# lowrank/aniso

Measured on AMD Instinct MI355X. Metric: GMRES matvec/s at 1M quad points (aniso.m block matvec, g=0.8, 45 mode-applies), higher is better.
Workload: dtype f64

## Files before the change

aniso_amd/csrc/aniso_op.hip:

```cpp
#include <algorithm>
#include <cmath>
#include <cstdlib>
#include <cstring>
#include <stdexcept>
#include <thread>

#include "aniso_op.hpp"
#include "kernels.hpp"

namespace aniso {

[[noreturn]] void throw_hip(hipError_t e, const char* file, int line) {
    throw std::runtime_error(std::string("HIP error ") + hipGetErrorName(e) + " (" + hipGetErrorString(e) + ") at " +
                             file + ":" + std::to_string(line));
}

#define HIP_CHECK(x)                                         \
    do {                                                     \
        hipError_t e__ = (x);                                \
        if (e__ != hipSuccess) throw_hip(e__, __FILE__, __LINE__); \
    } while (0)

DevBuf::~DevBuf() {
    if (p) (void)hipFree(p);
// ... 947 lines not shown
                      cf.Wc.as<double>(), cf.Wm.as<double>(), P};
    const int ntier = (int)plan.upTierTask.size() - 1;
    const bool upPartial = call.exch.oneX && call.exch.upPartial && phase != 0;
    const bool topFused = harmonic && (mask & kStageFar) && topFusedOn() && !upPartial && !win;
    const bool ringOn = hmRing > 0 && hm_ring_xl(K, plan.hmMaxLds, hmRing) >= 0;
    const bool hsSym = harmonic && plan.nearSymHsOn;
    const bool nearFused = topFused && overlapOn() && nearInTop && !ringOn && !hsSym && plan.nearCorrOk &&
                           near_hs_fusable((int)plan.leaves.size(), plan.nearMaxLeaf, plan.nsMax,
                                           dNearLoc.as<uint16_t>(), &nc, mask);
    const bool fork = harmonic && overlapOn() && !nearFused;
    const hipStream_t sn = fork ? side : s;
    const bool nearIn = harmonic && nearEarly && !nearFused && plan.nearCorrOk && (mask & kStageNear) &&
                        near_hs_fusable((int)plan.leaves.size(), plan.nearMaxLeaf, plan.nsMax,
                                        dNearLoc.as<uint16_t>(), &nc, mask);
    const bool oneX = call.exch.oneX && phase != 0;
    if (oneX && !(harmonic && nearIn))
        throw std::logic_error("one-collective exchange: the apply is not the harmonic one with its near field from the input");
    double* const fTw = nearIn ? nullptr : dFT.as<double>();
    double* const cTw = nearIn ? nullptr : dCT.as<double>();
    const int forkTier = phase == 0 && !topFused ? std::max(ntier - 1, 0) : plan.upLastLeafTier;
    UpTail tail;
    if (upPartial && call.exch.upTails) {
        tail.partOf = dXT0Part.as<int2>();
        const size_t sb = plan.xUpRoots.size() * 16 * kRank * K * sizeof(double);
        if (dXUpStage.bytes < sb) dXUpStage.alloc(sb);
        tail.stage = dXUpStage.as<double>();
        tail.cnt = dXUpCnt.as<unsigned>();
        tail.nroots = dXUpRoots.as<int>();
        tail.task = dXUpTask.as<int>();
        tail.rec = dXUpRec.as<double>();
        tail.nPeer = (int)oxRootParts;
        tail.peerOff = dOxRootSend.as<int64_t>();
        tail.buf = dOxSendBuf.as<double>();
    }
    auto upTier = [&](int k, const int* list, int ntask, const double* recv, double* send, const UpTail* tl = nullptr) {
        launch_up_tier(K, ntask, plan.upTierTask[k], list, plan.upTierMaxTask[k], dUpDesc.as<int4>(), dUpGrpFix.as<int>(),
                       dUpNode.as<int>(), dUpCode.as<int4>(), dUpGeom.as<double4>(), dUpLeaf.as<int2>(),
                       dPxT.as<double>(), dPyT.as<double>(), x, ldx, treeIn ? 1 : 0, dPerm.as<int>(), sigT,
                       dWT.as<double>(), fTw, cTw, P, dMult.as<double>(),
                       recv ? dXRootSlot.as<int>() : nullptr, recv, send ? dXSendSlot.as<int>() : nullptr, send, s,
                       topFused && k == 0 ? dTopCnt.as<unsigned>() : nullptr, tl);
        if (fork && !nearIn && k == forkTier) HIP_CHECK(hipEventRecord(evFork, s));
    };
    auto tierTasks = [&](int k) { return plan.upTierTask[k + 1] - plan.upTierTask[k]; };
    NearHsArgs nin{};
    if (nearIn) {
        nin.xin = x;
        nin.ldi = ldx;
        nin.treeIn = treeIn ? 1 : 0;
        nin.perm = dPerm.as<int>();
        nin.sigT = sigT;
        nin.wT = dWT.as<double>();
    }
    const bool nearUp = phase == 0 && nearIn && !fork && nearUpTier() && ntier >= 1 && !hsSym && K <= 5;
    if (nearUp) {
        nin.upMult = dMult.as<double>();
        nin.upGrp = dNearUpGrp.as<int>();
        nin.upP = P;
        nin.upNcx = dNcx.as<double>();
        nin.upNcy = dNcy.as<double>();
        nin.upNrx = dNrx.as<double>();
        nin.upNry = dNry.as<double>();
        nin.zeroCnt = topFused ? dTopCnt.as<unsigned>() : nullptr;
    }
    if (hsSym) {
        nin.nearSym = dHsSym.as<int2>();
        nin.colDst = dHsDst.as<int>();
        nin.selfRow = dNearSelfRow.as<uint16_t>();
        nin.nearPart = dNearPart.as<double>();
        nin.grpInPtr = dNearGrpInPtr.as<int>();
        nin.grpIn = dNearGrpIn.as<int>();
        nin.grpSlots = plan.nearGrpSlots;
    }
    const int64_t* const hmPtsPtr = (hsSym ? dHsPtsPtr : dNearPtsPtr).as<int64_t>();
    const int64_t* const hmKOff = (hsSym ? dHsKOff : dNearKOff).as<int64_t>();
    const uint16_t* const hmLoc = (hsSym ? dHsLoc : dNearLoc).as<uint16_t>();
    auto nearStage = [&] {
        if (fork) HIP_CHECK(hipStreamWaitEvent(side, evFork, 0));
        const int en = tr ? mark(sn) : -1;
        bool corrFused = false;
        if (harmonic) {
            corrFused = launch_near_hm(K, (int)plan.leaves.size(), plan.nearMaxLeaf, dLeafInfo.as<int4>(), hmPtsPtr,
                           dNearPts.as<int>(), hmKOff, dAttNear.as<double>(), dPxT.as<double>(), dPyT.as<double>(),
                           dSigDiag.as<double>(), hw, dFT.as<double>(), operm, obase, ldo, mask, scale, out, hmLoc,
                           dNsPtr.as<int64_t>(), dNsPts.as<int>(), plan.nsMax, plan.nearCorrOk ? &nc : nullptr,
                           nearWpe, sn, &nin, win);
        } else if (plan.nearPartTotal > 0) {
            for (int t = 0; t < nterm; ++t) {
                const int id = ids[t];
                const double sgn = (id % 2 == 0) ? 1.0 : -1.0;
                launch_near_sym(K, (int)plan.leaves.size(), dLeafInfo.as<int4>(), dNearPtsPtr.as<int64_t>(),
                                dNearPts.as<int>(), dNearKOff.as<int64_t>(), dNearSym.as<int2>(),
                                modes[id].Knear.as<double>(), dFT.as<double>(), mixes + (size_t)t * K * K, operm,
                                obase, ldo, maxNearS, mask, sgn, scale, t > 0 ? 1 : 0, dNearPart.as<double>(), out, s);
            }
        } else {
            launch_near(K, (int)plan.leaves.size(), plan.nearMaxLeaf, dLeafInfo.as<int4>(), dNearPtsPtr.as<int64_t>(),
                        dNearPts.as<int>(), dNearKOff.as<int64_t>(), tab, nterm, dFT.as<double>(), operm, obase, ldo,
                        mask, scale, 0, out, s);
        }
        const int e1 = tr ? mark(sn) : -1;
        span(4, en, e1);
        if (!corrFused)
            launch_corr(K, geo.d, plan.ownBegin, plan.ownEnd, dPerm.as<int>(), dIperm.as<int>(), dCT.as<double>(),
                        dFT.as<double>(), cf.Wc.as<double>(), cf.Wm.as<double>(), P, mask, scale, treeOut, ldo, out, sn);
        const int e2 = tm ? mark(sn) : -1;
        span(6, e1, e2);
        if (fork) HIP_CHECK(hipEventRecord(evJoin, side));
    };
    const bool clustered = harmonic && useClusters && !win;
    const int ncl = (int)plan.hmClPtr.size() - 1;
    HcArgs hca{dHmClPtr.as<int>(), dHmTgt.as<int>(), dHmPtr.as<int64_t>(), dHmNDir.as<int>(), dHmSrc.as<int>(),
                     dHmBlk.as<int>(), dHmSlot.as<int>(), dAttM2L.as<double>(), dNcx.as<double>(), dNcy.as<double>(),
                     dNrx.as<double>(), dNry.as<double>(), P, hw, dMult.as<double>(), dLocal.as<double>(),
                     dNodeGeo.as<double>()};
    hca.wpe = hmWpe;
    const bool halo = !plan.hmHaloNode.empty();
    if (halo) {
        const size_t hb = plan.hmHaloNode.size() * kRank * K * sizeof(double);
        if (dHmPart.bytes < hb) dHmPart.alloc(hb);
        hca.haloPtr = dHmHaloPtr.as<int>();
        hca.haloPos = dHmHaloPos.as<int>();
        hca.hpart = dHmPart.as<double>();
    }
    if (hmRing > 0) {
// ... 1871 lines not shown
```

aniso_amd/csrc/harmonic.hip:

```cpp
#include <hip/hip_runtime.h>

#include <algorithm>
#include <cstdlib>
#include <stdexcept>
#include <string>

#include "corr_point.hpp"
#include "device_common.hpp"
#include "hm_entry.hpp"
#include "up_task.hpp"

namespace aniso {

__device__ __forceinline__ double uniform_f64(double v) {
    const long long b = __double_as_longlong(v);
    const int lo = __builtin_amdgcn_readfirstlane((int)(b & 0xffffffffll));
    const int hi = __builtin_amdgcn_readfirstlane((int)(b >> 32));
    return __longlong_as_double(((long long)hi << 32) | (unsigned)lo);
}

__device__ __forceinline__ int xcd_tile(int bid, int nb) {
    const int x = bid & 7, per = nb >> 3, rem = nb & 7, j = bid >> 3;
    return x < rem ? x * (per + 1) + j : rem * (per + 1) + (x - rem) * per + j;
}
// ... 697 lines not shown
    __syncthreads();
    const bool ok = done != 0;
    __syncthreads();
    return ok;
}

template <int K>
__device__ __forceinline__ void top_ensure(const TopArgs& t, const UpArgs& u, int k, double* sm) {
    int j = k;
    while (j >= 1 && !top_poll(t, j, (unsigned)(t.blk0[j + 1] - t.blk0[j]))) --j;
    for (int jj = j + 1; jj <= k; ++jj) {
        const int nj = t.blk0[jj + 1] - t.blk0[jj];
        for (int i = 0; i < nj; ++i) {
            up_task<K>(t.task0[jj] + i, u.maxTask, u.desc, u.grpFix, u.node, u.code, u.geom, u.leafRange, u.pxT,
                       u.pyT, u.xin, u.ldi, u.treeIn, u.perm, u.sigT, u.wT, u.fT, u.cT, u.P, u.mult, u.rootSlot,
                       jj == 1 ? t.recv1 : nullptr, nullptr, nullptr, sm);
            asm volatile("s_waitcnt vmcnt(0)" ::: "memory");
            __syncthreads();
        }
        if (threadIdx.x == 0 && t.steals)
            __hip_atomic_fetch_add((gu32*)t.steals, (unsigned)nj, __ATOMIC_RELAXED, __HIP_MEMORY_SCOPE_AGENT);
    }
}

__device__ __forceinline__ void top_publish(unsigned* cnt, int k) {
    asm volatile("s_waitcnt vmcnt(0)" ::: "memory");
    __syncthreads();
    if (threadIdx.x == 0) {
        __builtin_amdgcn_fence(__ATOMIC_RELEASE, "agent");
        asm volatile("s_waitcnt vmcnt(0)" ::: "memory");
        __hip_atomic_fetch_add((gu32*)(cnt + k), 1u, __ATOMIC_RELAXED, __HIP_MEMORY_SCOPE_AGENT);
    }
}

template <bool TRACE>
__device__ __forceinline__ void top_mark(const TopArgs& t, int field) {
    if constexpr (!TRACE) return;
    __syncthreads();
    if (threadIdx.x == 0) {
        int64_t* r = t.trace + 4 * (int64_t)blockIdx.x;
        r[field] = (int64_t)__builtin_amdgcn_s_memrealtime();
        if (field == 0)
            r[3] = (int64_t)__builtin_amdgcn_s_getreg((4) | (0 << 6) | (31 << 11)) |
                   ((int64_t)__builtin_amdgcn_s_getreg((20) | (0 << 6) | (3 << 11)) << 32);
    }
}

template <int K, int NR, int D, bool XL, bool LR = false>
__device__ __forceinline__ void m2l_cluster_form(int cid, const HcArgs& a, double* sm) {
    if constexpr (D == 0) m2l_hc_cluster<K, NR, LR>(cid, a, sm);
    else m2l_hcr_cluster<K, NR, D, XL>(cid, a, sm);
}

template <int K, int U, int NR, bool FUSE, bool SYM = false, bool UP = false, bool OFF = false>
__device__ __forceinline__ void near_hs_group(int g, const NearHsArgs& n, double* tab, int i0 = 0, int b0 = 0);

template <int K, int NR, int WPE, int D, bool XL, bool TRACE = false, bool NEAR = false>
__global__ void __launch_bounds__(kHcThreads<WPE>) __attribute__((amdgpu_waves_per_eu(kHcWaves<WPE>)))
k_top_m2l_hc(UpArgs u, TopArgs t, HcArgs a, NearHsArgs n) {
    extern __shared__ double sm[];
    const int b = (int)blockIdx.x;
    top_mark<TRACE>(t, 0);
    if (b < t.nUp) {
        int k = 1;
        while (b >= t.blk0[k + 1]) ++k;
        if (k >= 2) top_ensure<K>(t, u, k - 1, sm);
        top_mark<TRACE>(t, 1);
        up_task<K>(t.task0[k] + (b - t.blk0[k]), u.maxTask, u.desc, u.grpFix, u.node, u.code, u.geom, u.leafRange,
                   u.pxT, u.pyT, u.xin, u.ldi, u.treeIn, u.perm, u.sigT, u.wT, u.fT, u.cT, u.P, u.mult, u.rootSlot,
                   k == 1 ? t.recv1 : nullptr, nullptr, nullptr, sm);
        top_publish(t.cnt, k);
        top_mark<TRACE>(t, 2);
        return;
    }
    const int cid = b - t.nUp;
    if constexpr (NEAR) {
        if (cid >= t.nCl) {
            top_mark<TRACE>(t, 1);
            near_hs_group<K, 4, 2, true>(cid - t.nCl, n, sm);
            top_mark<TRACE>(t, 2);
            return;
        }
    }
    const int w = t.clWait[cid];
    if (w > 0) {
        top_ensure<K>(t, u, w, sm);
        top_mark<TRACE>(t, 1);
        m2l_cluster_form<K, NR, D, XL, kHcLR<WPE>>(cid, a, sm);
        top_mark<TRACE>(t, 2);
        return;
    }
    top_mark<TRACE>(t, 1);
    m2l_cluster_form<K, NR, D, XL, kHcLR<WPE>>(cid, a, sm);
    top_mark<TRACE>(t, 2);
}


template <int K, int G, int U, int NR, bool XCD = false, bool OFF = false>
__global__ void __launch_bounds__(256) k_near_hm(int nl, const int4* __restrict__ leafInfo,
                                                 const int64_t* __restrict__ nearPtsPtr,
                                                 const int* __restrict__ nearPts, const int64_t* __restrict__ nearKOff,
                                                 const double* __restrict__ E, const double* __restrict__ pxT,
                                                 const double* __restrict__ pyT, const double* __restrict__ sigDiag,
                                                 HarmArg<OFF> hw, const double* __restrict__ fT,
                                                 const int* __restrict__ operm, int64_t obase, int64_t ldo,
                                                 int flags, double scale, double* __restrict__ out) {
    static_assert(G == 16 || G == 64, "leaf group of 16 or 64 lanes");
// ... 183 lines not shown
        double* LM = PT + (size_t)l * 16 * PW;
#pragma unroll
        for (int b = 0; b < K; ++b) LM[ln * K + b] = acc[b];
        if (active)
#pragma unroll
            for (int b = 0; b < K; ++b) n.upMult[((size_t)leafNode * kRank + ln) * K + b] = acc[b];
    }
    __syncthreads();
    double Rr[kRank];
    {
        const double* R2 = &P->R[threadIdx.x & 3][((threadIdx.x >> 2) & 15) * kRank];
#pragma unroll
        for (int rr = 0; rr < kRank; ++rr) Rr[rr] = threadIdx.x < 64 ? R2[rr] : 0.0;
    }
    {
        const int m = um, r = ur, c = uc;
        const double* x = PT + (size_t)(4 * m + c) * 16 * PW;
        double acc[K];
#pragma unroll
        for (int b = 0; b < K; ++b) acc[b] = 0.0;
#pragma unroll
        for (int rr = 0; rr < kRank; ++rr)
#pragma unroll
            for (int b = 0; b < K; ++b) acc[b] = __builtin_fma(Rc[rr], x[rr * K + b], acc[b]);
#pragma unroll
        for (int b = 0; b < K; ++b) acc[b] = quad_sum(acc[b]);
        if (c == 0) {
#pragma unroll
            for (int b = 0; b < K; ++b) {
                PM[(m * kRank + r) * K + b] = acc[b];
                n.upMult[((size_t)parentNode * kRank + r) * K + b] = acc[b];
            }
        }
    }
    __syncthreads();
    if (threadIdx.x < 64) {
        const int r = threadIdx.x >> 2, m = threadIdx.x & 3;
        const double* x = PM + (size_t)m * RK;
        double acc[K];
#pragma unroll
        for (int b = 0; b < K; ++b) acc[b] = 0.0;
#pragma unroll
        for (int rr = 0; rr < kRank; ++rr)
#pragma unroll
            for (int b = 0; b < K; ++b) acc[b] = __builtin_fma(Rr[rr], x[rr * K + b], acc[b]);
#pragma unroll
        for (int b = 0; b < K; ++b) acc[b] = quad_sum(acc[b]);
        if (m == 0)
#pragma unroll
            for (int b = 0; b < K; ++b) n.upMult[((size_t)rootNode * kRank + r) * K + b] = acc[b];
    }
}

template <int K, int U, int NR, bool FUSE, bool SYM, bool UP, bool OFF>
__device__ __forceinline__ void near_hs_group(const int g, const NearHsArgs& n, double* tab, int i0, int b0) {
    static_assert(!(OFF && (SYM || UP)), "the offset form: the plain staged near field");
    constexpr int KS = kStride<K>;
    constexpr int RW = kTabRow<K>;
    const int nl = n.nl;
    const int4* __restrict__ leafInfo = n.leafInfo;
    const int64_t* __restrict__ nearPtsPtr = n.nearPtsPtr;
    const uint16_t* __restrict__ nearLoc = n.nearLoc;
    const int64_t* __restrict__ nsPtr = n.nsPtr;
    const int* __restrict__ nsPts = n.nsPts;
    const int64_t* __restrict__ nearKOff = n.nearKOff;
    const double* __restrict__ E = n.E;
    const double* __restrict__ pxT = n.pxT;
    const double* __restrict__ pyT = n.pyT;
    const double* __restrict__ sigDiag = n.sigDiag;
    const HarmWeights& hw = n.hw;
    const double* __restrict__ fT = n.fT;
    const int* __restrict__ operm = n.operm;
    const int64_t obase = n.obase, ldo = n.ldo;
    const int flags = n.flags;
    const double scale = n.scale;
    double* __restrict__ out = n.out;
    const NearCorr& nc = n.nc;
    const bool nearOn = (flags & kStageNear) != 0;
    const bool fromIn = n.xin != nullptr;
    auto wcharges = [&](int64_t p, double (&f)[K]) {
        if (fromIn) {
            const double w = n.wT[p];
#pragma unroll
            for (int b = 0; b < K; ++b) f[b] = input_charge(n.xin, n.ldi, b, n.treeIn, n.perm, n.sigT, p) * w;
        } else {
            load_charges<K>(fT + (size_t)p * KS, f);
        }
    };
    const bool sym = SYM && nearOn;
    double* dslot = tab + (size_t)n.nsMax * RW;
    if (nearOn) {
        const int64_t r0 = nsPtr[g];
        const int nr = (int)(nsPtr[g + 1] - r0);
        for (int i = threadIdx.x; i < nr; i += blockDim.x) {
            const int64_t p = nsPts[r0 + i];
            double* row = tab + (size_t)i * RW;
            row[0] = pxT[p];
            row[1] = pyT[p];
            double f[K];
            wcharges(p, f);
#pragma unroll
            for (int v = 0; v < K; ++v) row[2 + v] = f[v];
        }
    }
#ifdef ANISO_NEAR_SYM_ATOMIC
    if (sym)
        for (int i = threadIdx.x; i < 256 * K; i += blockDim.x) dslot[i] = 0.0;
#endif
    __syncthreads();
    const int gl = threadIdx.x & 15;
    const int li = g * 16 + (int)(threadIdx.x >> 4);
    const bool active = li < nl;
    int4 info = make_int4(0, 0, 0, 0);
    int64_t pb = 0, koff = 0;
    if (active) {
        info = leafInfo[li];
        pb = nearPtsPtr[li];
        koff = nearKOff[li];
    }
    const int nT = info.z;
    const int S = !nearOn ? 0 : sym && active ? n.nearSym[li].x : info.w;
    const int64_t tb = info.y;
    const int nq = (nT + 3) >> 2;
    const int cstr = 2 * nq;
    const int rq = gl & 3, cph = gl >> 2;
    const bool rowOk = active && rq < nq;
    double tx[4], ty[4];
#pragma unroll
    for (int j = 0; j < 4; ++j) {
        const int t = min(4 * rq + j, max(nT - 1, 0));
        tx[j] = rowOk ? pxT[tb + t] : 0.0;
        ty[j] = rowOk ? pyT[tb + t] : 0.0;
    }
    double a[4][K];
#pragma unroll
    for (int j = 0; j < 4; ++j)
#pragma unroll
        for (int i = 0; i < K; ++i) a[j][i] = 0.0;
    if (rowOk) {
        const dbl2* kc = reinterpret_cast<const dbl2*>(E + koff) + 2 * rq;
        auto fetch = [&](int c0, dbl2 (&kk)[U][2], int (&ix)[U]) {
#pragma unroll
            for (int u = 0; u < U; ++u) {
                const int sc = c0 + u * 4;
                const bool ok = sc < S;
                const dbl2* p = kc + (size_t)min(sc, S - 1) * cstr;
                kk[u][0] = ok ? __builtin_nontemporal_load(p) : dbl2{0.0, 0.0};
                kk[u][1] = ok ? __builtin_nontemporal_load(p + 1) : dbl2{0.0, 0.0};
                ix[u] = nearLoc[pb + min(sc, S - 1)];
            }
        };
        auto step = [&](const dbl2 (&kk)[U][2], const int (&ix)[U]) {
#pragma unroll
            for (int u = 0; u < U; ++u) {
                const double* row = tab + (size_t)ix[u] * RW;
                const double sx = row[0], sy = row[1];
                double xw[K];
#pragma unroll
                for (int b = 0; b < K; ++b) xw[b] = hw.hw[b] * row[2 + b];
                const double e4[4] = {kk[u][0].x, kk[u][0].y, kk[u][1].x, kk[u][1].y};
#pragma unroll
                for (int j = 0; j < 4; ++j) {
                    const double dy = sy - ty[j];
                    if constexpr (!OFF) hm_entry<K, true, NR>(e4[j], sx - tx[j], dy * dy, xw, a[j]);
                }
                if constexpr (OFF) {
                    double dxs[4], dys[4];
#pragma unroll
                    for (int j = 0; j < 4; ++j) {
                        dxs[j] = sx - tx[j];
                        dys[j] = (sy - ty[j]) * (sy - ty[j]);
                    }
                    hm_rows_win<K, true, NR>(e4, dxs, dys, i0, b0, xw, a);
                }
            }
        };
        for (int c0 = cph; c0 < S; c0 += U * 4) {
            dbl2 kk[U][2];
            int ix[U];
            fetch(c0, kk, ix);
            step(kk, ix);
        }
    }
    if constexpr (SYM) if (sym && active) {
        constexpr int UC = 2;
        double xa[4][K];
#pragma unroll
        for (int j = 0; j < 4; ++j) {
            const int t = 4 * rq + j;
            const double* row = tab + (size_t)(n.selfRow[li] + min(t, max(nT - 1, 0))) * RW + 2;
#pragma unroll
            for (int b = 0; b < K; ++b) xa[j][b] = t < nT ? ((b & 1) ? -hw.hw[b] : hw.hw[b]) * row[b] : 0.0;
        }
        const dbl2* kc = reinterpret_cast<const dbl2*>(E + koff) + 2 * rq;
        const int S1 = n.nearSym[li].y;
        const int* __restrict__ dst = n.colDst + pb;
        for (int c0 = S + cph; c0 < S1; c0 += UC * 4) {
            dbl2 kk[UC][2];
            int ix[UC], dd[UC];
#pragma unroll
            for (int u = 0; u < UC; ++u) {
                const int sc = min(c0 + u * 4, S1 - 1);
                const bool ok = c0 + u * 4 < S1 && rq < nq;
                const dbl2* p = kc + (size_t)sc * cstr;
                kk[u][0] = ok ? __builtin_nontemporal_load(p) : dbl2{0.0, 0.0};
                kk[u][1] = ok ? __builtin_nontemporal_load(p + 1) : dbl2{0.0, 0.0};
                ix[u] = nearLoc[pb + sc];
                dd[u] = dst[sc];
            }
#pragma unroll
            for (int u = 0; u < UC; ++u) {
                if (c0 + u * 4 >= S1) break;
                const double* row = tab + (size_t)ix[u] * RW;
                const double sx = row[0], sy = row[1];
                double xw[K], ob[K];
#pragma unroll
                for (int b = 0; b < K; ++b) {
                    xw[b] = hw.hw[b] * row[2 + b];
                    ob[b] = 0.0;
                }
                const double e4[4] = {kk[u][0].x, kk[u][0].y, kk[u][1].x, kk[u][1].y};
#pragma unroll
                for (int j = 0; j < 4; ++j) {
                    const double dy = sy - ty[j];
                    hm_entry2<K, NR>(e4[j], sx - tx[j], dy * dy, xw, xa[j], a[j], ob);
                }
#pragma unroll
                for (int i = 0; i < K; ++i) ob[i] = quad_sum(ob[i]);
#pragma unroll
                for (int i = 0; i < K; ++i) {
                    if ((i & 3) != rq) continue;
                    const double v = (i & 1) ? -ob[i] : ob[i];
#ifdef ANISO_NEAR_SYM_ATOMIC
                    if (dd[u] < 0) atomicAdd(dslot + (size_t)(~dd[u]) * K + i, v);
#else
                    if (dd[u] < 0) dslot[(size_t)(~dd[u]) * K + i] = v;
#endif
                    else n.nearPart[(size_t)dd[u] * K + i] = hw.om[i] * v;
                }
            }
        }
    }
#pragma unroll
    for (int j = 0; j < 4; ++j)
#pragma unroll
        for (int i = 0; i < K; ++i) {
            double v = a[j][i];
            v += dpp_f64<0x124>(v);
            v += dpp_f64<0x128>(v);
            a[j][i] = v;
        }
    if (sym) __syncthreads();
    double fq[K];
#pragma unroll
    for (int i = 0; i < K; ++i) fq[i] = 0.0;
    if (rowOk) {
        const int t = 4 * rq + cph;
        double av[K];
#pragma unroll
        for (int i = 0; i < K; ++i) av[i] = cph == 0 ? a[0][i] : cph == 1 ? a[1][i] : cph == 2 ? a[2][i] : a[3][i];
#ifdef ANISO_NEAR_SYM_ATOMIC
        if (sym && t < nT) {
            const double* d = dslot + ((size_t)(li & 15) * 16 + t) * K;
#pragma unroll
            for (int i = 0; i < K; ++i) av[i] += d[i];
        }
        if (false) {
#else
        if (sym && t < nT) {
#endif
            const int q1 = n.grpInPtr[li + 1];
            for (int q = n.grpInPtr[li]; q < q1; ++q) {
                const double* d = dslot + ((size_t)n.grpIn[q] * 16 + t) * K;
#pragma unroll
                for (int i = 0; i < K; ++i) av[i] += d[i];
            }
        }
        if (t < nT) {
            const int64_t k = tb + t;
            double f[K];
            wcharges(k, f);
#pragma unroll
            for (int i = 0; i < K; ++i) fq[i] = f[i];
            const double sd = nearOn ? sigDiag[k] : 0.0;
            const int64_t oi = out_index(operm, obase, k);
            double cr[K];
            if constexpr (FUSE) {
                const uint16_t* rw = nc.rows + ((size_t)li * 16 + t) * 9;
                auto cval = [&](int64_t p, int r) {
                    return fromIn ? input_charge(n.xin, n.ldi, r, n.treeIn, n.perm, n.sigT, p)
                                  : nc.cT[(size_t)p * KS + r];
                };
                corr_point<1, K>(nc.perm[k], nc.P, nc.iperm, cval, nc.Wc, nc.Wm, flags,
                                 [&](int q9, int, int, double (&fc)[K]) {
                                     const double* row = tab + (size_t)rw[q9] * RW + 2;
#pragma unroll
                                     for (int b = 0; b < K; ++b) fc[b] = row[b];
                                 },
                                 cr);
            } else {
#pragma unroll
                for (int i = 0; i < K; ++i) cr[i] = 0.0;
            }
#pragma unroll
            for (int i = 0; i < K; ++i)
                out[(size_t)i * ldo + oi] =
                    __builtin_fma(hw.om[i] * scale, __builtin_fma(hw.dw[i] * sd, f[i], av[i]), cr[i] * scale);
        }
    }
    if constexpr (UP) near_up_tail<K>(g, active, nT, tb, info.x, n, fq, tab);
}

template <int K>
static size_t near_hs_lds(const NearHsArgs& n) {
    const size_t tab = (size_t)n.nsMax * kTabRow<K> * sizeof(double) +
                       (n.colDst ? (size_t)n.grpSlots * 16 * K * sizeof(double) : 0);
    return std::max(tab, n.upMult ? near_up_lds_doubles(K) * sizeof(double) : (size_t)0);
}

#ifndef ANISO_NEAR_SYM_WPE
#define ANISO_NEAR_SYM_WPE 1
#endif
template <bool OFF>
struct NearHsArg : NearHsArgs {};
template <>
struct NearHsArg<true> : NearHsArgs {
    int i0, b0;
};
static_assert(sizeof(NearHsArg<false>) == sizeof(NearHsArgs), "the flag-off kernels take NearHsArgs as it is");

template <int K, int U, int NR, bool FUSE, bool W4 = false, bool SYM = false, bool UP = false, bool OFF = false>
__global__ void __launch_bounds__(256) __attribute__((amdgpu_waves_per_eu(W4 ? 4 : SYM ? ANISO_NEAR_SYM_WPE : 1))) k_near_hs(NearHsArg<OFF> n) {
    extern __shared__ double tab[];
    if (n.zeroCnt && blockIdx.x == 0 && threadIdx.x <= kMaxTopTiers) n.zeroCnt[threadIdx.x] = 0u;
    if constexpr (OFF)
        near_hs_group<K, U, NR, FUSE, SYM, UP, true>(n.grpList ? n.grpList[blockIdx.x] : (int)blockIdx.x, n, tab, n.i0,
                                                     n.b0);
    else near_hs_group<K, U, NR, FUSE, SYM, UP>(n.grpList ? n.grpList[blockIdx.x] : (int)blockIdx.x, n, tab);
}



#define ANISO_HM_DISPATCH_K(k, CALL)                                                                    \
    switch (k) {                                                                                        \
        case 2: { constexpr int KK = 2; CALL; } break;                                                  \
        case 4: { constexpr int KK = 4; CALL; } break;                                                  \
        case 5: { constexpr int KK = 5; CALL; } break;                                                  \
        case 8: { constexpr int KK = 8; CALL; } break;                                                  \
        default: throw std::invalid_argument("harmonic apply: unsupported block count " + std::to_string(k)); \
    }

void launch_m2l_hm(int K, int ntgt, const int* tgt, const int64_t* ptr, const int* src, const int* blk, const double* E,
                   const double* ncx, const double* ncy, const double* nrx, const double* nry, const Params* P,
                   const HarmWeights& hw, const double* mult, double* local, hipStream_t s, const HarmWindow* win) {
    if (ntgt <= 0) return;
    const unsigned nb = blocks_for((int64_t)ntgt * kWave, 256);
    if (win) {
        if (K != kMaxRhs) throw std::invalid_argument("harmonic M2L: the offset form takes 8 blocks per pass");
        k_m2l_hm<kMaxRhs, 2, 2, 2, true><<<nb, 256, 0, s>>>(ntgt, 0, tgt, ptr, src, blk, E, ncx, ncy, nrx, nry, P,
                                                            harm_arg<true>(hw, win), mult, local);
        HIP_LAUNCH_CHECK();
        return;
    }
    ANISO_HM_DISPATCH_K(K, (k_m2l_hm<KK, 2, 2, 4><<<nb, 256, 0, s>>>(ntgt, 0, tgt, ptr, src, blk, E, ncx, ncy, nrx, nry,
                                                                      P, harm_arg<false>(hw, nullptr), mult, local)));
    HIP_LAUNCH_CHECK();
}

size_t m2l_hc_lds(int K, int maxCl, int depth, bool xl, int nw) {
    size_t b = (size_t)maxCl * kRank * K * sizeof(double);
    if (depth == 0 || xl) b += (size_t)nw * kRank * K * sizeof(double);
    if (depth == 0) return b;
    const size_t slot = 2048 + (size_t)kRank * K * 8 + 32;
    return b + (size_t)nw * depth * slot;
}

int hm_ring_depth() {
    const char* e = std::getenv("ANISO_HM_RING");
    const int v = e ? std::atoi(e) : 0;
    return v == 0 ? 0 : std::max(2, std::min(4, v));
}

int hm_ring_xl(int K, int maxCl, int depth) {
    if (K > kRingMaxK) return -1;
    if (const char* e = std::getenv("ANISO_HM_RING_XL")) return std::atoi(e) != 0 ? 1 : 0;
    return 3 * m2l_hc_lds(K, maxCl, depth, true, 4) <= 160 * 1024 ? 1 : -1;
}

#define ANISO_HM_DISPATCH_RING(d, CALL)                                            \
    switch (d) {                                                                   \
        case 0: { constexpr int DD = 0; CALL; } break;                             \
// ... 133 lines not shown
            auto f = near ? (t.trace ? k_top_m2l_hc<KK, 1, 3, 0, false, true, true>
                                     : k_top_m2l_hc<KK, 1, 3, 0, false, false, true>)
                          : (t.trace ? k_top_m2l_hc<KK, 1, 3, 0, false, true> : k_top_m2l_hc<KK, 1, 3, 0, false>);
            if (form == 6) f = t.trace ? k_top_m2l_hc<KK, 1, 6, 0, false, true> : k_top_m2l_hc<KK, 1, 6, 0, false>;
            if constexpr (KK <= kRingMaxK) {
                if (form == 4) f = t.trace ? k_top_m2l_hc<KK, 1, 4, 0, false, true> : k_top_m2l_hc<KK, 1, 4, 0, false>;
                if (form == 8) f = t.trace ? k_top_m2l_hc<KK, 1, 8, 0, false, true> : k_top_m2l_hc<KK, 1, 8, 0, false>;
            }
            set_lds(f, shm);
            f<<<nb, hm_threads(form), shm, s>>>(u, t, a, n);
        } else {
            auto f = xl ? (t.trace ? k_top_m2l_hc<KK, 1, 3, DD, true, true> : k_top_m2l_hc<KK, 1, 3, DD, true>)
                        : (t.trace ? k_top_m2l_hc<KK, 1, 2, DD, false, true> : k_top_m2l_hc<KK, 1, 2, DD, false>);
            set_lds(f, shm);
            f<<<nb, 256, shm, s>>>(u, t, a, n);
        }
    })));
    HIP_LAUNCH_CHECK();
}

static bool near_hs_staged(int nl, int maxLeaf, int nsMax, const uint16_t* nearLoc) {
    return nl > 0 && maxLeaf <= 16 && nsMax > 0 && nearLoc && (size_t)nsMax * kTabRow<8> * sizeof(double) <= 64 * 1024;
}


bool near_hs_fusable(int nl, int maxLeaf, int nsMax, const uint16_t* nearLoc, const NearCorr* corr, int flags) {
    return near_hs_staged(nl, maxLeaf, nsMax, nearLoc) && corr && corr->rows && (flags & kStageNear);
}

bool launch_near_hm(int K, int nl, int maxLeaf, const int4* leafInfo, const int64_t* nearPtsPtr, const int* nearPts,
                    const int64_t* nearKOff, const double* E, const double* pxT, const double* pyT,
                    const double* sigDiag, const HarmWeights& hw, const double* fT, const int* operm, int64_t obase,
                    int64_t ldo, int flags, double scale, double* out, const uint16_t* nearLoc, const int64_t* nsPtr,
                    const int* nsPts, int nsMax, const NearCorr* corr, int wpe, hipStream_t s, const NearHsArgs* in,
                    const HarmWindow* win) {
    if (nl <= 0) return false;
    if (win && (K != kMaxRhs || (in && (in->upMult || in->colDst))))
        throw std::invalid_argument("harmonic near field: the offset form takes 8 blocks per pass, directed storage");
    if (near_hs_staged(nl, maxLeaf, nsMax, nearLoc)) {
        unsigned ng = (unsigned)((nl + 15) / 16);
        const bool fuse = near_hs_fusable(nl, maxLeaf, nsMax, nearLoc, corr, flags);
        NearHsArgs n{nl, nsMax, leafInfo, nearPtsPtr, nearLoc, nsPtr, nsPts, nearKOff, E, pxT, pyT, sigDiag, hw,
                     fT, operm, obase, ldo, flags, scale, out, fuse ? *corr : NearCorr{}};
        if (in && in->xin) {
            if (!fuse) throw std::invalid_argument("near field from the input: only with its fused corrections");
            n.xin = in->xin;
            n.ldi = in->ldi;
            n.treeIn = in->treeIn;
            n.perm = in->perm;
            n.sigT = in->sigT;
            n.wT = in->wT;
        }
        if (in && in->upMult) {
            if (!fuse || in->colDst)
                throw std::invalid_argument("near field with the up tier: not the staged directed kernel with its table");
            n.upMult = in->upMult;
            n.upGrp = in->upGrp;
            n.upP = in->upP;
            n.upNcx = in->upNcx;
            n.upNcy = in->upNcy;
            n.upNrx = in->upNrx;
            n.upNry = in->upNry;
            n.zeroCnt = in->zeroCnt;
        }
        if (in && in->grpList) {
            n.grpList = in->grpList;
            n.ngrp = in->ngrp;
            ng = (unsigned)in->ngrp;
            if (ng == 0) return fuse;
        }
        if (in && in->colDst) {
            if (!in->nearSym || !in->selfRow || !in->nearPart || !in->grpInPtr)
                throw std::invalid_argument("symmetric staged near field: missing lists");
            n.nearSym = in->nearSym;
            n.colDst = in->colDst;
            n.selfRow = in->selfRow;
            n.nearPart = in->nearPart;
            n.grpInPtr = in->grpInPtr;
            n.grpIn = in->grpIn;
            n.grpSlots = in->grpSlots;
        }
        if (win) {
            NearHsArg<true> na;
            static_cast<NearHsArgs&>(na) = n;
            na.i0 = win->i0;
            na.b0 = win->b0;
            const size_t shm = near_hs_lds<kMaxRhs>(n);
            auto f = fuse ? k_near_hs<kMaxRhs, 2, 2, true, false, false, false, true>
                          : k_near_hs<kMaxRhs, 2, 2, false, false, false, false, true>;
            f<<<ng, 256, shm, s>>>(na);
            HIP_LAUNCH_CHECK();
            return fuse;
        }
        NearHsArg<false> na;
        static_cast<NearHsArgs&>(na) = n;
        ANISO_HM_DISPATCH_K(K, ({
            const size_t shm = near_hs_lds<KK>(n);
            auto f = n.colDst ? (fuse ? k_near_hs<KK, 4, 2, true, false, true> : k_near_hs<KK, 4, 2, false, false, true>)
                     : fuse ? (n.upMult ? k_near_hs<KK, 2, 2, true, true, false, true>
                               : wpe == 4 ? k_near_hs<KK, 2, 2, true, true> : k_near_hs<KK, 2, 2, true>)
                            : (wpe == 4 ? k_near_hs<KK, 2, 2, false, true> : k_near_hs<KK, 2, 2, false>);
            f<<<ng, 256, shm, s>>>(na);
        }));
        HIP_LAUNCH_CHECK();
        return fuse;
    }
#define ANISO_NEAR_HM(G)                                                                                          \
    if (win)                                                                                                      \
        k_near_hm<kMaxRhs, G, 2, 2, false, true><<<blocks_for((int64_t)nl * G, 256), 256, 0, s>>>(                \
            nl, leafInfo, nearPtsPtr, nearPts, nearKOff, E, pxT, pyT, sigDiag, harm_arg<true>(hw, win), fT, operm, \
            obase, ldo, flags, scale, out);                                                                       \
    else                                                                                                          \
        ANISO_HM_DISPATCH_K(K, (k_near_hm<KK, G, 4, 2><<<blocks_for((int64_t)nl * G, 256), 256, 0, s>>>(           \
                                   nl, leafInfo, nearPtsPtr, nearPts, nearKOff, E, pxT, pyT, sigDiag,              \
                                   harm_arg<false>(hw, nullptr), fT, operm, obase, ldo, flags, scale, out)))
    if (in && in->colDst) throw std::invalid_argument("symmetric near storage needs the staged near field");
    if (in && in->grpList) throw std::invalid_argument("a near-field group subset needs the staged near field");
    if (maxLeaf <= 16) {
        ANISO_NEAR_HM(16);
    } else {
        ANISO_NEAR_HM(64);
    }
#undef ANISO_NEAR_HM
    HIP_LAUNCH_CHECK();
    return false;
}

}
```

aniso_amd/csrc/host_tree.cpp:

```cpp
#include <algorithm>
#include <atomic>
#include <cstdlib>
#include <functional>
#include <cmath>
#include <stdexcept>
#include <thread>
#include <unordered_map>

#include "host.hpp"

namespace aniso {

namespace {

struct Builder {
    Tree& t;
    const double* x;
    const double* y;
    int rank, maxLevelArg;
    std::vector<int> tmp;

    int new_node(int level, int slot) {
        t.parent.push_back(-1);
        t.level.push_back(level);
// ... 423 lines not shown
    if (nranks != 1 || nsMax <= 0 || ng == 0 || leaves.size() != 16 * ng || upTierTask.size() < 2 ||
        (size_t)(upTierTask[1] - upTierTask[0]) != ng)
        return;
    std::vector<int> taskOf(t.nn, -1);
    for (int k = upTierTask[0]; k < upTierTask[1]; ++k) taskOf[upTaskRoot[k]] = k;
    for (size_t g = 0; g < ng; ++g) {
        const int* L = leaves.data() + 16 * g;
        if (t.parent[L[0]] < 0 || t.parent[t.parent[L[0]]] < 0) return;
        const int A = t.parent[t.parent[L[0]]];
        const int k = taskOf[A];
        if (k < 0 || upTaskPtr[k + 1] - upTaskPtr[k] != 21) return;
        std::array<int, 25> G{};
        int found = 0;
        for (int c = 0; c < 16; ++c) {
            const int p = t.parent[L[c]];
            if (t.parent[p] != A || !t.isLeaf[L[c]] || t.isEmpty[L[c]]) return;
            int m = -1, q = -1;
            for (int i = 0; i < 4; ++i) {
                if (t.child[A][i] == p) m = i;
                if (t.child[p][i] == L[c]) q = i;
            }
            if (m < 0 || q < 0 || m != c / 4) return;
            G[c] = (m << 2) | q;
            found |= 1 << (4 * m + q);
        }
        if (found != 0xFFFF) return;
        for (int m = 0; m < 4; ++m) {
            G[16 + m] = m;
            G[20 + m] = t.child[A][m];
        }
        G[24] = A;
        nearUpGrp.insert(nearUpGrp.end(), G.begin(), G.end());
    }
    nearUpOk = true;
}

void Plan::buildNearHs(const Tree& t, const std::vector<int>& leafIdx) {
    hsPtsPtr.assign(1, 0);
    hsLoc.clear();
    hsKOff.clear();
    hsSym.clear();
    hsSrcPtr.assign(1, 0);
    hsSrc.clear();
    hsDst.clear();
    nearSelfRow.clear();
    hsKTotal = 0;
    hsPartTotal = 0;
    hsStored = 0;
    nearGrpInPtr.assign(1, 0);
    nearGrpIn.clear();
    nearGrpSlots = 0;
    nearSymHsOn = nearSymHs && !nearSymmetric && nearMaxLeaf <= 16 && !leaves.empty() &&
                  nsPtr.size() == (leaves.size() + 15) / 16 + 1 &&
                  (size_t)nsMax * 11 * 8 <= 64 * 1024;
    if (!nearSymHsOn) return;
    std::vector<std::vector<int>> inRef(leaves.size()), grpIn(16);
    std::vector<int> u, dir, can;
    for (size_t g0 = 0; g0 < leaves.size(); g0 += 16) {
        const size_t g1 = std::min(leaves.size(), g0 + 16);
        int q = 0;
        for (auto& v : grpIn) v.clear();
        u.assign(nsPts.begin() + nsPtr[g0 / 16], nsPts.begin() + nsPtr[g0 / 16 + 1]);
        auto row = [&](int64_t pos) {
            auto it = std::lower_bound(u.begin(), u.end(), (int)pos);
            if (it == u.end() || *it != (int)pos) throw std::logic_error("staged near field: source not in its table");
            return (uint16_t)(it - u.begin());
        };
        for (size_t li = g0; li < g1; ++li) {
            const int i = leaves[li];
            dir.clear();
            can.clear();
            for (int64_t k = t.uPtr[i]; k < t.uPtr[i + 1]; ++k) {
                const int b = t.uIdx[k];
                if (t.isEmpty[b]) continue;
                if (b != i && leafIdx[b] >= 0) {
                    if (i < b) can.push_back(b);
                    continue;
                }
                dir.push_back(b);
            }
            for (int64_t k = t.wPtr[i]; k < t.wPtr[i + 1]; ++k)
                if (!t.isEmpty[t.wIdx[k]]) dir.push_back(t.wIdx[k]);
            hsKOff.push_back(hsKTotal);
            int S = 0;
            for (int b : dir) {
                hsSrc.push_back(b);
                for (int64_t u0 = 0; u0 < t.count[b]; ++u0) {
                    hsLoc.push_back(row(t.begin[b] + u0));
                    hsDst.push_back(0);
                }
                S += (int)t.count[b];
            }
            const int Sdir = S;
            for (int b : can) {
                const int lb = leafIdx[b];
                if (lb / 16 == (int)li / 16 && q < kNearGrpSlots) {
                    grpIn[lb % 16].push_back(q);
#ifdef ANISO_NEAR_SYM_ATOMIC
                    for (int64_t u0 = 0; u0 < t.count[b]; ++u0) hsDst.push_back(~(int)((lb % 16) * 16 + u0));
#else
                    for (int64_t u0 = 0; u0 < t.count[b]; ++u0) hsDst.push_back(~(int)(q * 16 + u0));
#endif
                    ++q;
                } else {
                    inRef[lb].push_back((int)hsPartTotal);
                    for (int64_t u0 = 0; u0 < t.count[b]; ++u0) hsDst.push_back((int)(hsPartTotal + u0));
                    hsPartTotal += t.count[b];
                }
                hsSrc.push_back(b);
                for (int64_t u0 = 0; u0 < t.count[b]; ++u0) hsLoc.push_back(row(t.begin[b] + u0));
                S += (int)t.count[b];
            }
            hsSym.push_back({Sdir, S});
            hsKTotal += (int64_t)S * ((t.count[i] + 3) & ~(int64_t)3);
            hsStored += (int64_t)S * t.count[i];
            hsPtsPtr.push_back((int64_t)hsLoc.size());
            hsSrcPtr.push_back((int64_t)hsSrc.size());
            nearSelfRow.push_back(row(t.begin[i]));
        }
        for (size_t li = g0; li < g1; ++li) {
            const auto& v = grpIn[li - g0];
            nearGrpIn.insert(nearGrpIn.end(), v.begin(), v.end());
            nearGrpInPtr.push_back((int)nearGrpIn.size());
        }
        nearGrpSlots = std::max(nearGrpSlots, q);
#ifdef ANISO_NEAR_SYM_ATOMIC
        nearGrpSlots = 16;
#endif
    }
    if (hsPartTotal > ((int64_t)1 << 31) - 1) throw std::invalid_argument("near partials overflow");
    nearInPtr.assign(1, 0);
    nearInOff.clear();
    for (auto& v : inRef) {
        nearInOff.insert(nearInOff.end(), v.begin(), v.end());
        nearInPtr.push_back((int)nearInOff.size());
    }
}


static std::vector<std::vector<int>> task_levels(const Tree& t, int root, int bottom,
                                                 const std::function<bool(int)>& keep) {
    std::vector<std::vector<int>> lv{{root}};
    while (t.level[lv.back()[0]] < bottom) {
        std::vector<int> next;
        for (int n : lv.back())
            if (!t.isLeaf[n])
                for (int q = 0; q < 4; ++q) {
                    const int c = t.child[n][q];
                    if (c >= 0 && keep(c)) next.push_back(c);
                }
        if (next.empty()) break;
        lv.push_back(std::move(next));
    }
    return lv;
}

void Plan::buildUpTasks(const Tree& t) {
    std::vector<int> slotOf(t.nn, -1);
    auto keep = [&](int n) { return !t.isEmpty[n]; };
    upTierTask.assign(1, 0);
    upTaskRoot.clear();
    upTaskPtr.assign(1, 0);
    upGrpPtr.assign(1, 0);
    upGrp.clear();
    upNode.clear();
    upCode.clear();
    upDesc.clear();
    upGrpFix.clear();
    upGeom.clear();
    upLeaf.clear();
    upMaxTask = 1;
    upTierMaxTask.assign(tierRootLevel.size(), 1);
    for (size_t k = 0; k < tierRootLevel.size(); ++k) {
        for (int r = 0; r < t.nn; ++r) {
            if (t.level[r] != tierRootLevel[k] || t.isEmpty[r]) continue;
            auto lv = task_levels(t, r, tierBottomLevel[k], keep);
            const int base = (int)upNode.size();
            for (int L = (int)lv.size() - 1; L >= 0; --L) {
                upGrp.push_back((int)upNode.size());
                for (int n : lv[L]) {
                    slotOf[n] = (int)upNode.size() - base;
// ... 606 lines not shown
```

Baseline: 859.5.

## Make symmetric near-field default to LDS atomics with staged self sources

```diff
diff --git a/aniso_amd/csrc/aniso_op.hip b/aniso_amd/csrc/aniso_op.hip
--- a/aniso_amd/csrc/aniso_op.hip
+++ b/aniso_amd/csrc/aniso_op.hip
@@ -1023,7 +1023,8 @@
         nin.sigT = sigT;
         nin.wT = dWT.as<double>();
     }
-    const bool nearUp = phase == 0 && nearIn && !fork && nearUpTier() && ntier >= 1 && !hsSym && K <= 5;
+    const bool hsDet = hsSym && deterministicOn();
+    const bool nearUp = phase == 0 && nearIn && !fork && nearUpTier() && ntier >= 1 && !hsDet && K <= 5;
     if (nearUp) {
         nin.upMult = dMult.as<double>();
         nin.upGrp = dNearUpGrp.as<int>();
@@ -1041,7 +1042,7 @@
         nin.nearPart = dNearPart.as<double>();
         nin.grpInPtr = dNearGrpInPtr.as<int>();
         nin.grpIn = dNearGrpIn.as<int>();
-        nin.grpSlots = plan.nearGrpSlots;
+        nin.grpSlots = hsDet ? std::max(plan.nearGrpSlots, 1) : 0;
     }
     const int64_t* const hmPtsPtr = (hsSym ? dHsPtsPtr : dNearPtsPtr).as<int64_t>();
     const int64_t* const hmKOff = (hsSym ? dHsKOff : dNearKOff).as<int64_t>();
diff --git a/aniso_amd/csrc/harmonic.hip b/aniso_amd/csrc/harmonic.hip
--- a/aniso_amd/csrc/harmonic.hip
+++ b/aniso_amd/csrc/harmonic.hip
@@ -773,7 +773,7 @@
     else m2l_hcr_cluster<K, NR, D, XL>(cid, a, sm);
 }
 
-template <int K, int U, int NR, bool FUSE, bool SYM = false, bool UP = false, bool OFF = false>
+template <int K, int U, int NR, bool FUSE, bool SYM = false, bool UP = false, bool OFF = false, bool DET = false>
 __device__ __forceinline__ void near_hs_group(int g, const NearHsArgs& n, double* tab, int i0 = 0, int b0 = 0);
 
 template <int K, int NR, int WPE, int D, bool XL, bool TRACE = false, bool NEAR = false>
@@ -1063,9 +1063,10 @@
     }
 }
 
-template <int K, int U, int NR, bool FUSE, bool SYM, bool UP, bool OFF>
+template <int K, int U, int NR, bool FUSE, bool SYM, bool UP, bool OFF, bool DET>
 __device__ __forceinline__ void near_hs_group(const int g, const NearHsArgs& n, double* tab, int i0, int b0) {
     static_assert(!(OFF && (SYM || UP)), "the offset form: the plain staged near field");
+    static_assert(!DET || (SYM && !UP), "the slot-ordered sums: symmetric storage, without the up tail");
     constexpr int KS = kStride<K>;
     constexpr int RW = kTabRow<K>;
     const int nl = n.nl;
@@ -1100,6 +1101,7 @@
     };
     const bool sym = SYM && nearOn;
     double* dslot = tab + (size_t)n.nsMax * RW;
+    double* xself = dslot + 256 * K;
     if (nearOn) {
         const int64_t r0 = nsPtr[g];
         const int nr = (int)(nsPtr[g + 1] - r0);
@@ -1114,11 +1116,6 @@
             for (int v = 0; v < K; ++v) row[2 + v] = f[v];
         }
     }
-#ifdef ANISO_NEAR_SYM_ATOMIC
-    if (sym)
-        for (int i = threadIdx.x; i < 256 * K; i += blockDim.x) dslot[i] = 0.0;
-#endif
-    __syncthreads();
     const int gl = threadIdx.x & 15;
     const int li = g * 16 + (int)(threadIdx.x >> 4);
     const bool active = li < nl;
@@ -1130,6 +1127,18 @@
         koff = nearKOff[li];
     }
     const int nT = info.z;
+    __syncthreads();
+    if constexpr (SYM && !DET) {
+        if (sym) {
+            const double* row = tab + (size_t)((active ? n.selfRow[li] : 0) + min(gl, max(nT - 1, 0))) * RW + 2;
+#pragma unroll
+            for (int b = 0; b < K; ++b) {
+                dslot[(size_t)threadIdx.x * K + b] = 0.0;
+                xself[(size_t)threadIdx.x * K + b] = gl < nT ? ((b & 1) ? -hw.hw[b] : hw.hw[b]) * row[b] : 0.0;
+            }
+            __syncthreads();
+        }
+    }
     const int S = !nearOn ? 0 : sym && active ? n.nearSym[li].x : info.w;
     const int64_t tb = info.y;
     const int nq = (nT + 3) >> 2;
@@ -1195,14 +1204,17 @@
     }
     if constexpr (SYM) if (sym && active) {
         constexpr int UC = 2;
-        double xa[4][K];
-#pragma unroll
-        for (int j = 0; j < 4; ++j) {
-            const int t = 4 * rq + j;
-            const double* row = tab + (size_t)(n.selfRow[li] + min(t, max(nT - 1, 0))) * RW + 2;
-#pragma unroll
-            for (int b = 0; b < K; ++b) xa[j][b] = t < nT ? ((b & 1) ? -hw.hw[b] : hw.hw[b]) * row[b] : 0.0;
-        }
+        double xr[DET ? 4 : 1][K];
+        if constexpr (DET) {
+#pragma unroll
+            for (int j = 0; j < 4; ++j) {
+                const int t = 4 * rq + j;
+                const double* row = tab + (size_t)(n.selfRow[li] + min(t, max(nT - 1, 0))) * RW + 2;
+#pragma unroll
+                for (int b = 0; b < K; ++b) xr[j][b] = t < nT ? ((b & 1) ? -hw.hw[b] : hw.hw[b]) * row[b] : 0.0;
+            }
+        }
+        const double* xs = xself + ((size_t)(threadIdx.x >> 4) * 16 + 4 * rq) * K;
         const dbl2* kc = reinterpret_cast<const dbl2*>(E + koff) + 2 * rq;
         const int S1 = n.nearSym[li].y;
         const int* __restrict__ dst = n.colDst + pb;
@@ -1234,7 +1246,8 @@
 #pragma unroll
                 for (int j = 0; j < 4; ++j) {
                     const double dy = sy - ty[j];
-                    hm_entry2<K, NR>(e4[j], sx - tx[j], dy * dy, xw, xa[j], a[j], ob);
+                    if constexpr (DET) hm_entry2<K, NR>(e4[j], sx - tx[j], dy * dy, xw, xr[j], a[j], ob);
+                    else hm_entry2<K, NR>(e4[j], sx - tx[j], dy * dy, xw, xs + j * K, a[j], ob);
                 }
 #pragma unroll
                 for (int i = 0; i < K; ++i) ob[i] = quad_sum(ob[i]);
@@ -1242,12 +1255,11 @@
                 for (int i = 0; i < K; ++i) {
                     if ((i & 3) != rq) continue;
                     const double v = (i & 1) ? -ob[i] : ob[i];
-#ifdef ANISO_NEAR_SYM_ATOMIC
-                    if (dd[u] < 0) atomicAdd(dslot + (size_t)(~dd[u]) * K + i, v);
-#else
-                    if (dd[u] < 0) dslot[(size_t)(~dd[u]) * K + i] = v;
-#endif
-                    else n.nearPart[(size_t)dd[u] * K + i] = hw.om[i] * v;
+                    if (dd[u] >= 0) n.nearPart[(size_t)dd[u] * K + i] = hw.om[i] * v;
+                    else if constexpr (DET) dslot[(size_t)((~dd[u] >> 8) * 16 + (~dd[u] & 15)) * K + i] = v;
+                    else
+                        __hip_atomic_fetch_add(dslot + (size_t)(~dd[u] & 255) * K + i, v, __ATOMIC_RELAXED,
+                                               __HIP_MEMORY_SCOPE_WORKGROUP);
                 }
             }
         }
@@ -1270,16 +1282,12 @@
         double av[K];
 #pragma unroll
         for (int i = 0; i < K; ++i) av[i] = cph == 0 ? a[0][i] : cph == 1 ? a[1][i] : cph == 2 ? a[2][i] : a[3][i];
-#ifdef ANISO_NEAR_SYM_ATOMIC
-        if (sym && t < nT) {
+        if (SYM && !DET && sym && t < nT) {
             const double* d = dslot + ((size_t)(li & 15) * 16 + t) * K;
 #pragma unroll
             for (int i = 0; i < K; ++i) av[i] += d[i];
         }
-        if (false) {
-#else
-        if (sym && t < nT) {
-#endif
+        if (DET && sym && t < nT) {
             const int q1 = n.grpInPtr[li + 1];
             for (int q = n.grpInPtr[li]; q < q1; ++q) {
                 const double* d = dslot + ((size_t)n.grpIn[q] * 16 + t) * K;
@@ -1325,13 +1333,10 @@
 template <int K>
 static size_t near_hs_lds(const NearHsArgs& n) {
     const size_t tab = (size_t)n.nsMax * kTabRow<K> * sizeof(double) +
-                       (n.colDst ? (size_t)n.grpSlots * 16 * K * sizeof(double) : 0);
+                       (n.colDst ? (size_t)(n.grpSlots > 0 ? n.grpSlots * 16 : 2 * 256) * K * sizeof(double) : 0);
     return std::max(tab, n.upMult ? near_up_lds_doubles(K) * sizeof(double) : (size_t)0);
 }
 
-#ifndef ANISO_NEAR_SYM_WPE
-#define ANISO_NEAR_SYM_WPE 1
-#endif
 template <bool OFF>
 struct NearHsArg : NearHsArgs {};
 template <>
@@ -1340,14 +1345,16 @@
 };
 static_assert(sizeof(NearHsArg<false>) == sizeof(NearHsArgs), "the flag-off kernels take NearHsArgs as it is");
 
-template <int K, int U, int NR, bool FUSE, bool W4 = false, bool SYM = false, bool UP = false, bool OFF = false>
-__global__ void __launch_bounds__(256) __attribute__((amdgpu_waves_per_eu(W4 ? 4 : SYM ? ANISO_NEAR_SYM_WPE : 1))) k_near_hs(NearHsArg<OFF> n) {
+template <int K, int U, int NR, bool FUSE, bool W4 = false, bool SYM = false, bool UP = false, bool OFF = false,
+          bool DET = false>
+__global__ void __launch_bounds__(256) __attribute__((amdgpu_waves_per_eu(W4 ? 4 : SYM && !DET ? 3 : 1))) k_near_hs(NearHsArg<OFF> n) {
     extern __shared__ double tab[];
     if (n.zeroCnt && blockIdx.x == 0 && threadIdx.x <= kMaxTopTiers) n.zeroCnt[threadIdx.x] = 0u;
     if constexpr (OFF)
         near_hs_group<K, U, NR, FUSE, SYM, UP, true>(n.grpList ? n.grpList[blockIdx.x] : (int)blockIdx.x, n, tab, n.i0,
                                                      n.b0);
-    else near_hs_group<K, U, NR, FUSE, SYM, UP>(n.grpList ? n.grpList[blockIdx.x] : (int)blockIdx.x, n, tab);
+    else
+        near_hs_group<K, U, NR, FUSE, SYM, UP, false, DET>(n.grpList ? n.grpList[blockIdx.x] : (int)blockIdx.x, n, tab);
 }
 
 
@@ -1587,8 +1594,8 @@
             n.wT = in->wT;
         }
         if (in && in->upMult) {
-            if (!fuse || in->colDst)
-                throw std::invalid_argument("near field with the up tier: not the staged directed kernel with its table");
+            if (!fuse || (in->colDst && (in->grpSlots > 0 || K > 5)))
+                throw std::invalid_argument("near field with the up tier: not the staged kernel with its table and corrections");
             n.upMult = in->upMult;
             n.upGrp = in->upGrp;
             n.upP = in->upP;
@@ -1607,6 +1614,7 @@
         if (in && in->colDst) {
             if (!in->nearSym || !in->selfRow || !in->nearPart || !in->grpInPtr)
                 throw std::invalid_argument("symmetric staged near field: missing lists");
+            if (K > 5) throw std::invalid_argument("symmetric staged near field: at most 5 blocks");
             n.nearSym = in->nearSym;
             n.colDst = in->colDst;
             n.selfRow = in->selfRow;
@@ -1631,10 +1639,18 @@
         static_cast<NearHsArgs&>(na) = n;
         ANISO_HM_DISPATCH_K(K, ({
             const size_t shm = near_hs_lds<KK>(n);
-            auto f = n.colDst ? (fuse ? k_near_hs<KK, 4, 2, true, false, true> : k_near_hs<KK, 4, 2, false, false, true>)
-                     : fuse ? (n.upMult ? k_near_hs<KK, 2, 2, true, true, false, true>
-                               : wpe == 4 ? k_near_hs<KK, 2, 2, true, true> : k_near_hs<KK, 2, 2, true>)
-                            : (wpe == 4 ? k_near_hs<KK, 2, 2, false, true> : k_near_hs<KK, 2, 2, false>);
+            auto f = fuse ? (n.upMult ? k_near_hs<KK, 2, 2, true, true, false, true>
+                             : wpe == 4 ? k_near_hs<KK, 2, 2, true, true> : k_near_hs<KK, 2, 2, true>)
+                          : (wpe == 4 ? k_near_hs<KK, 2, 2, false, true> : k_near_hs<KK, 2, 2, false>);
+            if constexpr (KK <= 5) {
+                if (n.colDst)
+                    f = n.grpSlots > 0
+                            ? (fuse ? k_near_hs<KK, 2, 2, true, false, true, false, false, true>
+                                    : k_near_hs<KK, 2, 2, false, false, true, false, false, true>)
+                            : fuse ? (n.upMult ? k_near_hs<KK, 2, 2, true, false, true, true>
+                                               : k_near_hs<KK, 2, 2, true, false, true>)
+                                   : k_near_hs<KK, 2, 2, false, false, true>;
+            }
             f<<<ng, 256, shm, s>>>(na);
         }));
         HIP_LAUNCH_CHECK();
diff --git a/aniso_amd/csrc/host_tree.cpp b/aniso_amd/csrc/host_tree.cpp
--- a/aniso_amd/csrc/host_tree.cpp
+++ b/aniso_amd/csrc/host_tree.cpp
@@ -499,10 +499,16 @@
     nearGrpSlots = 0;
     nearSymHsOn = nearSymHs && !nearSymmetric && nearMaxLeaf <= 16 && !leaves.empty() &&
                   nsPtr.size() == (leaves.size() + 15) / 16 + 1 &&
-                  (size_t)nsMax * 11 * 8 <= 64 * 1024;
+                  (size_t)nsMax * 11 * 8 <= 64 * 1024 &&
+                  (size_t)nsMax * 7 * 8 + (size_t)kNearGrpSlots * 16 * 5 * 8 <= 64 * 1024;
     if (!nearSymHsOn) return;
     std::vector<std::vector<int>> inRef(leaves.size()), grpIn(16);
     std::vector<int> u, dir, can;
+    auto owns = [&](int i, int b) {
+        if (t.ncx[i] != t.ncx[b]) return t.ncx[i] < t.ncx[b];
+        if (t.ncy[i] != t.ncy[b]) return t.ncy[i] < t.ncy[b];
+        return i < b;
+    };
     for (size_t g0 = 0; g0 < leaves.size(); g0 += 16) {
         const size_t g1 = std::min(leaves.size(), g0 + 16);
         int q = 0;
@@ -521,7 +527,7 @@
                 const int b = t.uIdx[k];
                 if (t.isEmpty[b]) continue;
                 if (b != i && leafIdx[b] >= 0) {
-                    if (i < b) can.push_back(b);
+                    if (owns(i, b)) can.push_back(b);
                     continue;
                 }
                 dir.push_back(b);
@@ -543,11 +549,7 @@
                 const int lb = leafIdx[b];
                 if (lb / 16 == (int)li / 16 && q < kNearGrpSlots) {
                     grpIn[lb % 16].push_back(q);
-#ifdef ANISO_NEAR_SYM_ATOMIC
-                    for (int64_t u0 = 0; u0 < t.count[b]; ++u0) hsDst.push_back(~(int)((lb % 16) * 16 + u0));
-#else
-                    for (int64_t u0 = 0; u0 < t.count[b]; ++u0) hsDst.push_back(~(int)(q * 16 + u0));
-#endif
+                    for (int64_t u0 = 0; u0 < t.count[b]; ++u0) hsDst.push_back(~(int)(q << 8 | (lb % 16) << 4 | u0));
                     ++q;
                 } else {
                     inRef[lb].push_back((int)hsPartTotal);
@@ -571,9 +573,6 @@
             nearGrpInPtr.push_back((int)nearGrpIn.size());
         }
         nearGrpSlots = std::max(nearGrpSlots, q);
-#ifdef ANISO_NEAR_SYM_ATOMIC
-        nearGrpSlots = 16;
-#endif
     }
     if (hsPartTotal > ((int64_t)1 << 31) - 1) throw std::invalid_argument("near partials overflow");
     nearInPtr.assign(1, 0);
```

After: 859.8 (median of 4 runs). No clear change (+0.0%).
